# zendesk/min-tfs-client

Hardware: NVIDIA H100
Metric: TensorProto encode+decode GB/s (higher is better)
Workload: dtype u8

## Files before the change

include/b200tfs.h:

```cpp
#ifndef B200TFS_H_
#define B200TFS_H_

#include <stddef.h>
#include <stdint.h>

#ifdef __cplusplus
extern "C" {
#endif

#define B200TFS_ABI_VERSION 2

#define B200TFS_OK 0
#define B200TFS_E_DTYPE (-1)
#define B200TFS_E_SHAPE (-2)
#define B200TFS_E_SIZE (-3)
#define B200TFS_E_PARSE (-4)
#define B200TFS_E_CUDA (-5)
#define B200TFS_E_TOOBIG (-6)
#define B200TFS_E_ARG (-7)
#define B200TFS_E_NONCANONICAL (-8)
#define B200TFS_E_RANGE (-9)
#define B200TFS_E_KEY (-10)
#define B200TFS_E_SPILL (-11)

// ... 216 lines not shown
  int64_t dims[B200TFS_MAX_RANK];
  uint64_t bytes;
  int32_t status;
  int32_t bad_rec;
  uint8_t pad_bits[16];
} b200tfs_pad_key;
int b200tfs_padded_layout(const void* wire_host, int32_t n, const uint64_t* rec_off, const uint64_t* rec_len, int32_t n_keys,
                          b200tfs_pad_key* keys, int32_t cast);
int b200tfs_decode_padded(b200tfs_ctx* ctx, const void* arena_dev, int32_t n, const uint64_t* rec_off, const uint64_t* rec_len,
                          int32_t n_keys, const b200tfs_pad_key* keys);
int b200tfs_decode_padded_host_async(b200tfs_ctx* ctx, const void* wire_host, int32_t n, const uint64_t* rec_off,
                                     const uint64_t* rec_len, int32_t n_keys, const b200tfs_pad_key* keys);
int b200tfs_padded_results(b200tfs_ctx* ctx, int32_t n, int32_t n_keys, b200tfs_output* outs, b200tfs_model_spec* specs,
                           int32_t* rec_status);

int b200tfs_capture_begin(b200tfs_ctx* ctx);
int b200tfs_capture_end(b200tfs_ctx* ctx, void** graph_exec);
int b200tfs_graph_launch(b200tfs_ctx* ctx, void* graph_exec);
int b200tfs_graph_destroy(void* graph_exec);
int b200tfs_wait_event(b200tfs_ctx* ctx, void* ev);

int b200tfs_encode_requests_host(b200tfs_ctx* ctx, int32_t n, const b200tfs_request* reqs,
                                 void* wire_host, uint64_t wire_cap, uint64_t* rec_off,
                                 uint64_t* rec_len);
int b200tfs_encode_requests_host_async(b200tfs_ctx* ctx, int32_t n, const b200tfs_request* reqs,
                                       void* wire_host, uint64_t wire_cap, uint64_t* rec_off,
                                       uint64_t* rec_len);
int b200tfs_decode_responses_host_async(b200tfs_ctx* ctx, const void* wire_host, int32_t n,
                                        const uint64_t* rec_off, const uint64_t* rec_len,
                                        void* dst_host, uint64_t dst_stride);
int b200tfs_pipelined_calls(b200tfs_ctx* ctx, uint64_t* count);
int b200tfs_direct_calls(b200tfs_ctx* ctx, uint64_t* count);
int b200tfs_set_pipeline(b200tfs_ctx* ctx, uint64_t min_bytes, int32_t max_slices);
int b200tfs_encode_tensor_protos_host(b200tfs_ctx* ctx, int32_t n, const b200tfs_tensor* tensors,
                                      void* wire_host, uint64_t wire_cap, uint64_t* rec_off,
                                      uint64_t* rec_len);
int b200tfs_parse_responses_host(b200tfs_ctx* ctx, const void* wire_host, int32_t n,
                                 const uint64_t* rec_off, const uint64_t* rec_len, int32_t max_outputs,
                                 b200tfs_output* outs, int32_t* n_outs, b200tfs_model_spec* specs,
                                 int32_t* rec_status);
int b200tfs_parse_tensor_protos_host(b200tfs_ctx* ctx, const void* wire_host, int32_t n,
                                     const uint64_t* rec_off, const uint64_t* rec_len,
                                     b200tfs_output* outs, int32_t* rec_status);
int b200tfs_unpack_outputs_host(b200tfs_ctx* ctx, int32_t m, const b200tfs_output* outs,
                                const uint64_t* out_rec_off, void* const* dst_host,
                                const int32_t* dst_dtype, int32_t* status);

#define B200TFS_F_BROADCAST 0x10u
typedef struct b200tfs_feature {
  const void* data;
  int32_t src_dtype;
  uint32_t flags;
  int64_t row_elems;
  const char* key;
  int64_t key_len;
} b200tfs_feature;

typedef struct b200tfs_example_request {
  const char* model_name;
  int64_t model_name_len;
  int32_t has_version;
  int32_t order;
  int64_t version;
  int64_t n_examples;
  int32_t n_features;
  int32_t flags;
// ... 30 lines not shown
```

min-tfs-client_b200/csrc/codec_host.cpp:

```cpp
#include <cuda_runtime.h>
#include <stdarg.h>
#include <stdio.h>
#include <stdlib.h>
#include <string.h>

#include <algorithm>
#include <string>
#include <unordered_map>
#include <vector>

#include "../../include/b200tfs.h"
#include "example_walk.h"
#include "frame.h"
#include "kernels.h"
#include "plan.h"
#include "tpl.h"
#include "walker.h"
#include "wire.h"

using namespace b200tfs;

static thread_local char g_err[512] = "";

static int fail(int code, const char* fmt, ...) {
// ... 32 lines not shown
  int32_t dtype = 0;
  void* tile_val = nullptr;
  void* group_sum = nullptr;
  void* total = nullptr;
};

struct b200tfs_ctx {
  int device = 0;
  int sm_count = 132;
  cudaStream_t stream = nullptr;
  cudaStream_t own_stream = nullptr;
  cudaStream_t aux_stream = nullptr;
  cudaStream_t d2h_stream = nullptr;
  static constexpr int kPipeMax = 8;
  cudaEvent_t pipe_ev[2 * kPipeMax + 2] = {};
  uint64_t pipe_min = 1ull << 20;
  int pipe_max = 4;
  uint64_t pipelined_calls = 0;
  uint64_t direct_calls = 0;
  bool opt_direct_out = true;
  Growable guard_dev;
  uint32_t decode_cast = 0;
  uint32_t decode_varints = 0;
  bool fused_varints = false;
  Growable vdec_dev;
  Slot slots[kSlots];
  int next_slot = 0;
  Growable scratch_dev;
  Growable scratch_host;
  Growable stage_dev;
  Growable arena_dev;
  uint64_t launches = 0;
  uint32_t tile_bytes_override = 0;
  bool capturing = false;
  std::vector<Slot*> graph_slots;
  Growable fused_host;
  void* tpl_dev = nullptr;
  uint32_t tpl_flip = 0;
  TplInline* tpl_pinned = nullptr;
  TplInline tpl_known{};
  uint32_t serial = 0;
  cudaEvent_t tpl_event = nullptr;
  bool tpl_event_pending = false;
  bool opt_no_inline = false;
  uint64_t stage_shift = 0;
  int32_t fused_n = 0;
  std::vector<int32_t> pending_status;
  Growable measured_dev;
  uint64_t measured_used = 0;
  std::unordered_map<const void*, MeasuredTensor> measured;
  Growable spill_dev;
  std::vector<SpillEntry> spill_host;
  uint32_t spill_per_rec = 16;
  uint32_t spill_last_per = 0;
  int32_t spill_last_n = 0;
  Growable gather_dev;
  Growable enc_host;
  int32_t enc_n = 0;
  bool has_graphs = false;
  struct KeyResults {
    int32_t n = 0, k = 0;
    uint8_t* dst[B200TFS_CONCAT_MAX_KEYS] = {};
    uint64_t vouts = 0, vstat = 0, specs = 0, status = 0;
  };
  Growable concat_dev;
  KeyResults concat_res;
// ... 397 lines not shown

struct VarJob {
  const uint8_t* src;
  uint8_t* dst;
  uint64_t n_elems;
  uint64_t packed_len;
  int32_t src_dtype;
};

struct PlanBuilder {
  std::vector<MoveItem> items;
  std::vector<SmallItem> smalls;
  std::vector<uint8_t> blob;
  std::vector<VarJob> varjobs;
  uint64_t large_bytes = 0;
  const uint32_t* guard = nullptr;
  uint32_t guard_div = 1;
  bool independent = false;

  void header(uint8_t* dst, size_t blob_off, size_t n) {
    while (n) {
      uint32_t k = (uint32_t)std::min<size_t>(n, kSmallMax);
      smalls.push_back(SmallItem{(uint64_t)blob_off, dst, k, OP_COPY | OP_FLAG_BLOB, 0, 0});
      dst += k; blob_off += k; n -= k;
    }
  }
  void payload(const uint8_t* src, uint8_t* dst, uint64_t n_out, uint32_t op, uint32_t glen = 0, uint32_t gstride = 0) {
    if (!n_out) return;
    if (n_out <= kSmallMax) smalls.push_back(SmallItem{(uint64_t)(uintptr_t)src, dst, (uint32_t)n_out, op, glen, gstride});
    else { items.push_back(MoveItem{src, dst, n_out, op, 0, glen, gstride}); large_bytes += n_out; }
  }
};

uint32_t pick_vec_per_tile(const b200tfs_ctx* c, uint64_t large_bytes, uint64_t max_tile = 65536) {
  uint64_t tile = c->tile_bytes_override;
  if (!tile) {
    uint64_t target_tiles = (uint64_t)c->sm_count * 8;
    tile = (large_bytes + target_tiles - 1) / target_tiles;
    tile = (tile + 32767) & ~32767ull;
    tile = std::min<uint64_t>(std::max<uint64_t>(tile, 32768), max_tile);
  }
  tile = std::max<uint64_t>(tile & ~31ull, 32);
  return (uint32_t)(tile / 16);
}

struct BuiltPlan {
  PlanHeader ph{};
  uint8_t inline_buf[kInlinePlanBytes];
  const uint8_t* host_img = nullptr;
  uint8_t* plan_dev = nullptr;
  uint64_t image = 0;
  Slot* slot = nullptr;
};

int build_plan(b200tfs_ctx* c, PlanBuilder& pb, bool force_dev, BuiltPlan* bp) {
  const uint32_t vpt = pick_vec_per_tile(c, pb.large_bytes);
  uint64_t n_tiles = 0;
  uint32_t uniform = 0;
  bool is_uniform = !pb.items.empty();
  for (auto& it : pb.items) {
    uint64_t t = tiles_for_host(it.n_out, vpt);
    if (n_tiles + t > 0x7FFFFFFFull) return fail(B200TFS_E_TOOBIG, "batch needs more than 2^31 tiles");
    it.n_tiles = (uint32_t)t;
    if (&it == &pb.items[0]) uniform = (uint32_t)t; else if (t != uniform) is_uniform = false;
    n_tiles += t;
  }
  if (!is_uniform) uniform = 0;
  PlanHeader& ph = bp->ph;
  ph = PlanHeader{};
  ph.n_items = (uint32_t)pb.items.size();
  ph.n_tiles = (uint32_t)n_tiles;
  ph.n_small = (uint32_t)pb.smalls.size();
  ph.uniform_tpi = uniform;
  ph.vec_per_tile = vpt;
  ph.guard = pb.guard; ph.guard_div = pb.guard_div ? pb.guard_div : 1u;
  ph.independent = pb.independent ? 1u : 0u;
  const PlanGeometry g = plan_geometry(pb.items.size(), uniform ? 0 : n_tiles, pb.smalls.size());
  ph.off_items = (uint32_t)g.off_items; ph.off_tiles = (uint32_t)g.off_tiles; ph.off_small = (uint32_t)g.off_small;
  Layout P{g.end};
  const uint64_t off_blob = P.take(pb.blob.size(), 1);
  const uint64_t image = P.take(0);
  if (image > 0xFFFFFFFFull) return fail(B200TFS_E_TOOBIG, "plan image larger than 4 GiB");
  bp->image = image;
  uint8_t* img;
  const bool inl = !force_dev && image <= kInlinePlanBytes;
  if (inl) img = bp->inline_buf;
  else {
    int rc = claim_slot(c, image, &bp->slot);
    if (rc) return rc;
    img = (uint8_t*)bp->slot->host.p;
  }
  bp->host_img = img;
  memcpy(img, &ph, sizeof ph);
  if (!pb.items.empty()) memcpy(img + ph.off_items, pb.items.data(), pb.items.size() * sizeof(MoveItem));
  if (!uniform && n_tiles) {
    TileRef* tr = (TileRef*)(img + ph.off_tiles);
    uint32_t g = 0;
    for (uint32_t i = 0; i < pb.items.size(); ++i)
      for (uint32_t t = 0; t < pb.items[i].n_tiles; ++t) tr[g++] = TileRef{i, t};
  }
  SmallItem* sm = (SmallItem*)(img + ph.off_small);
  for (size_t i = 0; i < pb.smalls.size(); ++i) {
    sm[i] = pb.smalls[i];
    if (sm[i].op & OP_FLAG_BLOB) sm[i].src += off_blob;
  }
  if (!pb.blob.empty()) memcpy(img + off_blob, pb.blob.data(), pb.blob.size());
  if (!inl) {
    int rc = upload_slot(c, bp->slot, image);
    if (rc) return rc;
    bp->plan_dev = (uint8_t*)bp->slot->dev.p;
  }
  return B200TFS_OK;
}

int launch_built_plan(b200tfs_ctx* c, BuiltPlan& bp) {
  CU(launch_move(bp.plan_dev, bp.host_img, (uint32_t)bp.image, bp.ph.n_tiles, bp.ph.n_small, c->stream));
  c->launches += 1;
  if (bp.slot && bp.slot->done && !c->capturing) { CU(cudaEventRecord(bp.slot->done, c->stream)); bp.slot->pending = true; }
  return B200TFS_OK;
}

int launch_plan(b200tfs_ctx* c, PlanBuilder& pb) {
  if (pb.items.empty() && pb.smalls.empty()) return B200TFS_OK;
  BuiltPlan bp;
  int rc = build_plan(c, pb, false, &bp);
  if (rc) return rc;
  return launch_built_plan(c, bp);
}

inline uint64_t place_record(uint64_t cursor, uint64_t largest_payload_off) {
  uint64_t slot = (cursor + 255) & ~255ull;
  uint64_t pad = (128 - (largest_payload_off & 127)) & 127;
  return slot + pad;
}

int plan_tensor(const b200tfs_tensor& t, const TensorLayout& L, uint8_t* dst_payload, PlanBuilder& pb) {
  if (!L.payload_len) return B200TFS_OK;
  if (L.varint) {
    pb.varjobs.push_back(VarJob{(const uint8_t*)t.data, dst_payload, L.n_elems, L.payload_len, t.src_dtype});
    return B200TFS_OK;
  }
  pb.payload((const uint8_t*)t.data, dst_payload, L.payload_len, L.op);
  return B200TFS_OK;
}

int run_varjobs(b200tfs_ctx* c, PlanBuilder& pb);

struct RequestLayout {
  std::vector<TensorLayout> tl;
// ... 1189 lines not shown
    if (direct) c->direct_calls += 1;
    else for (int i = 0; i < n; ++i) rec_off[i] -= lo;
    return B200TFS_OK;
  }
  if ((rc = grow_dev(c, c->arena_dev, need))) return rc;
  if ((rc = b200tfs_encode_requests(c, n, rq.data(), c->arena_dev.p, c->arena_dev.cap, rec_off, rec_len))) return rc;
  const uint64_t lo = rec_off[0], hi = rec_off[n - 1] + rec_len[n - 1];
  if (hi - lo > wire_cap) return fail(B200TFS_E_SIZE, "wire buffer too small: need %llu bytes", (unsigned long long)(hi - lo));
  CU(cudaMemcpyAsync(wire_host, (uint8_t*)c->arena_dev.p + lo, hi - lo, cudaMemcpyDeviceToHost, c->stream));
  for (int i = 0; i < n; ++i) rec_off[i] -= lo;
  return B200TFS_OK;
}

int b200tfs_pipelined_calls(b200tfs_ctx* c, uint64_t* count) {
  if (!c || !count) return fail(B200TFS_E_ARG, "bad arguments");
  *count = c->pipelined_calls;
  return B200TFS_OK;
}

int b200tfs_direct_calls(b200tfs_ctx* c, uint64_t* count) {
  if (!c || !count) return fail(B200TFS_E_ARG, "bad arguments");
  *count = c->direct_calls;
  return B200TFS_OK;
}

int b200tfs_set_pipeline(b200tfs_ctx* c, uint64_t min_bytes, int32_t max_slices) {
  if (!c) return fail(B200TFS_E_ARG, "ctx is NULL");
  if (min_bytes && (max_slices < 2 || max_slices > b200tfs_ctx::kPipeMax)) return fail(B200TFS_E_ARG, "max_slices must be in [2, %d]", b200tfs_ctx::kPipeMax);
  c->pipe_min = min_bytes;
  if (min_bytes) c->pipe_max = max_slices;
  return B200TFS_OK;
}

int b200tfs_encode_requests_host(b200tfs_ctx* c, int32_t n, const b200tfs_request* reqs, void* wire_host, uint64_t wire_cap,
                                 uint64_t* rec_off, uint64_t* rec_len) {
  int rc = b200tfs_encode_requests_host_async(c, n, reqs, wire_host, wire_cap, rec_off, rec_len);
  if (rc) return rc;
  CU(cudaStreamSynchronize(c->stream));
  return B200TFS_OK;
}

static int stage_wire(b200tfs_ctx* c, const void* wire_host, int32_t n, const uint64_t* rec_off, const uint64_t* rec_len, uint64_t* span,
                      uint64_t shift = 0, bool copy = true) {
  uint64_t hi = 0;
  for (int i = 0; i < n; ++i) hi = std::max(hi, rec_off[i] + rec_len[i]);
  int rc = grow_dev(c, c->stage_dev, hi + 64);
  if (rc) return rc;
  c->stage_shift = shift;
  if (hi && copy) CU(cudaMemcpyAsync((uint8_t*)c->stage_dev.p + shift, wire_host, hi, cudaMemcpyHostToDevice, c->stream));
  *span = hi;
  return B200TFS_OK;
}

int b200tfs_parse_responses_host(b200tfs_ctx* c, const void* wire_host, int32_t n, const uint64_t* rec_off, const uint64_t* rec_len,
                                 int32_t max_outputs, b200tfs_output* outs, int32_t* n_outs, b200tfs_model_spec* specs,
                                 int32_t* rec_status) {
  if (!c || n < 0 || (n && (!wire_host || !rec_off || !rec_len))) return fail(B200TFS_E_ARG, "bad arguments");
  if (n == 0) return B200TFS_OK;
  CU(cudaSetDevice(c->device));
  uint64_t span;
  int rc = stage_wire(c, wire_host, n, rec_off, rec_len, &span);
  if (rc) return rc;
  return parse_common(c, c->stage_dev.p, n, rec_off, rec_len, max_outputs, false, outs, n_outs, specs, rec_status);
}

int b200tfs_parse_tensor_protos_host(b200tfs_ctx* c, const void* wire_host, int32_t n, const uint64_t* rec_off, const uint64_t* rec_len,
// ... 220 lines not shown
ConcatLayout concat_layout(uint64_t n, uint64_t n_keys, uint64_t tile_cap, uint64_t var_tile_cap) {
  const PlanGeometry g = plan_geometry(n * n_keys * B200TFS_MAX_RUNS, tile_cap, 0);
  const VarPlanLayout V = var_plan_layout(n, var_tile_cap);
  Layout R;
  ConcatLayout L;
  L.outs = R.take(sizeof(b200tfs_output) * n * (kFusedMaxOutputs + 1), 256);
  L.nouts = R.take(4 * n, 256);
  L.specs = R.take(sizeof(b200tfs_model_spec) * n, 256);
  L.status = R.take(4 * n, 256);
  L.spill = R.take(4 * n, 256);
  L.kst = R.take(4 * n * n_keys, 256);
  L.match = R.take(4 * n * n_keys, 256);
  L.plan = R.take(g.end, 256);
  L.plan_tiles = g.off_tiles;
  L.vouts = R.take(sizeof(b200tfs_output) * n * kFusedMaxOutputs, 256);
  L.vnouts = R.take(4 * n, 256);
  L.vstatus = R.take(4 * n, 256);
  L.var = R.take(V.bytes, 256);
  L.var_status = L.var + V.status;
  L.bytes = R.end;
  return L;
}
}

int b200tfs_decode_concat(b200tfs_ctx* c, const void* arena_dev, int32_t n, const uint64_t* rec_off, const uint64_t* rec_len,
                          int32_t n_keys, const b200tfs_concat_key* keys) {
  if (!c || n <= 0 || !arena_dev || !rec_off || !rec_len) return fail(B200TFS_E_ARG, "bad arguments");
  int rc = concat_check_keys(n_keys, keys);
  if (rc) return rc;
  for (int k = 0; k < n_keys; ++k) if (keys[k].dst_cap && !keys[k].dst) return fail(B200TFS_E_ARG, "key %d: dst is NULL", k);
  if (!c->capturing) CU(cudaSetDevice(c->device));
  uint64_t wire_total = 0, tile_cap = 0, var_tile_cap = 0;
  for (int i = 0; i < n; ++i) wire_total += rec_len[i];
  const uint32_t vpt = pick_vec_per_tile(c, c->decode_cast ? wire_total / 2 : wire_total);
  for (int i = 0; i < n; ++i) {
    tile_cap += concat_record_tile_bound(rec_len[i], 16ull * vpt, (uint32_t)n_keys);
    var_tile_cap += var_record_tile_bound(rec_len[i]);
  }
  if (tile_cap > 0x7FFFFFFFull || var_tile_cap > 0x7FFFFFFFull) return fail(B200TFS_E_TOOBIG, "batch needs more than 2^31 tiles");
  const ConcatLayout L = concat_layout((uint64_t)n, (uint64_t)n_keys, tile_cap, var_tile_cap);
  if (L.plan_tiles > 0xFFFFFFFFull) return fail(B200TFS_E_TOOBIG, "plan image larger than 4 GiB");
  if ((rc = grow_dev(c, c->concat_dev, L.bytes))) return rc;
  uint64_t key_bytes = 0;
  for (int k = 0; k < n_keys; ++k) key_bytes += (uint64_t)keys[k].key_len;
  Layout K;
  const uint64_t o_off = K.take(8ull * n), o_len = K.take(8ull * n), o_keys = K.take(sizeof(ConcatKeyDev) * n_keys), o_kb = K.take(key_bytes);
  Slot* slot;
  uint8_t* sd;
  rc = upload_image(c, K.end, {{o_off, rec_off, 8ull * n}, {o_len, rec_len, 8ull * n}}, &sd, &slot, [&](uint8_t* h, uint8_t* dev) {
    uint64_t at = o_kb;
    for (int k = 0; k < n_keys; ++k) {
      ConcatKeyDev kd{dev + at, (uint8_t*)keys[k].dst, keys[k].dst_cap, (uint32_t)keys[k].key_len, 0u};
      memcpy(h + o_keys + sizeof(ConcatKeyDev) * k, &kd, sizeof kd);
      if (keys[k].key_len) memcpy(h + at, keys[k].key, (size_t)keys[k].key_len);
      at += (uint64_t)keys[k].key_len;
    }
  });
  if (rc) return rc;
  for (int k = 0; k < n_keys; ++k) c->concat_res.dst[k] = (uint8_t*)keys[k].dst;
  uint8_t* d = (uint8_t*)c->concat_dev.p;
  const uint64_t* off_dev = (const uint64_t*)(sd + o_off);
  CU(launch_parse_responses((const uint8_t*)arena_dev, off_dev, (const uint64_t*)(sd + o_len), n, kFusedMaxOutputs, (b200tfs_output*)(d + L.outs),
                            (int32_t*)(d + L.nouts), (b200tfs_model_spec*)(d + L.specs), (int32_t*)(d + L.status), nullptr, 0u,
                            (uint32_t*)(d + L.spill), c->stream));
  ConcatPlan cp{};
  cp.w = (const uint8_t*)arena_dev; cp.rec_off = off_dev; cp.outs = (const b200tfs_output*)(d + L.outs);
  cp.n_outs = (const int32_t*)(d + L.nouts); cp.rec_status = (const int32_t*)(d + L.status);
// ... 185 lines not shown
```

min-tfs-client_b200/csrc/kernels.cu:

```cuda
#include <cuda_bf16.h>
#include <cuda_fp16.h>
#include <cuda_runtime.h>
#include <stdint.h>
#include <stdlib.h>
#include <string.h>

#include <algorithm>
#include <utility>

#include "frame.h"
#include "kernels.h"
#include "plan.h"
#include "tpl.h"
#include "example_walk.h"
#include "walker.h"
#include "wire.h"

namespace b200tfs {

__device__ __forceinline__ uint4 ld_stream(const uint8_t* p) {
  uint4 r;
  asm volatile("ld.global.nc.L1::no_allocate.v4.u32 {%0,%1,%2,%3}, [%4];"
               : "=r"(r.x), "=r"(r.y), "=r"(r.z), "=r"(r.w) : "l"(p));
  return r;
}
__device__ __forceinline__ uint4 ld_reuse(const uint8_t* p) {
  uint4 r;
  asm volatile("ld.global.nc.v4.u32 {%0,%1,%2,%3}, [%4];"
               : "=r"(r.x), "=r"(r.y), "=r"(r.z), "=r"(r.w) : "l"(p));
  return r;
}
__device__ __forceinline__ void st_stream(uint8_t* p, const uint4& v) {
  asm volatile("st.global.L1::no_allocate.v4.u32 [%0], {%1,%2,%3,%4};"
               :: "l"(p), "r"(v.x), "r"(v.y), "r"(v.z), "r"(v.w) : "memory");
}

__device__ __forceinline__ void pdl_launch_dependents() { asm volatile("griddepcontrol.launch_dependents;" ::: "memory"); }
__device__ __forceinline__ void pdl_wait_prior_grids() { asm volatile("griddepcontrol.wait;" ::: "memory"); }

__device__ __forceinline__ uint32_t bool_norm_word(uint32_t w) {
  uint32_t t = ((w & 0x7F7F7F7Fu) + 0x7F7F7F7Fu) | w;
  return (t >> 7) & 0x01010101u;
}

template <uint32_t OP>
__device__ __forceinline__ uint4 fix_vec(uint4 v) {
  if (OP == OP_QUIET_SRC || OP == OP_QUIET_DST) {
    v.x = quiet_f32(v.x); v.y = quiet_f32(v.y); v.z = quiet_f32(v.z); v.w = quiet_f32(v.w);
  } else if (OP == OP_BOOL) {
    v.x = bool_norm_word(v.x); v.y = bool_norm_word(v.y); v.z = bool_norm_word(v.z); v.w = bool_norm_word(v.w);
  }
  return v;
}

template <int Q>
__device__ __forceinline__ uint4 shift_pair(const uint4& lo, const uint4& hi, uint32_t s) {
  const uint32_t w[8] = {lo.x, lo.y, lo.z, lo.w, hi.x, hi.y, hi.z, hi.w};
  uint4 o;
  o.x = __funnelshift_r(w[Q + 0], w[Q + 1], s);
  o.y = __funnelshift_r(w[Q + 1], w[Q + 2], s);
  o.z = __funnelshift_r(w[Q + 2], w[Q + 3], s);
  o.w = __funnelshift_r(w[Q + 3], w[Q + 4], s);
  return o;
}

__device__ __forceinline__ uint32_t ld_u32_bytes(const uint8_t* p) {
  return (uint32_t)p[0] | ((uint32_t)p[1] << 8) | ((uint32_t)p[2] << 16) | ((uint32_t)p[3] << 24);
// ... 154 lines not shown
    case 1: return body_shifted_q<OP, 1>(S, dst, n, s, mid);
    case 2: return body_shifted_q<OP, 2>(S, dst, n, s, mid);
    default: return body_shifted_q<OP, 3>(S, dst, n, s, mid);
  }
}

template <bool BF>
__device__ __forceinline__ void body_widen(const uint8_t* __restrict__ src, uint8_t* __restrict__ dst, uint32_t units) {
  constexpr uint32_t kU = 8;
  for (uint32_t base = 0; base < units; base += kU * kMoveThreads) {
    uint4 h[kU];
#pragma unroll
    for (uint32_t i = 0; i < kU; ++i) {
      const uint32_t u = base + i * kMoveThreads + threadIdx.x;
      h[i] = make_uint4(0, 0, 0, 0);
      if (u < units) h[i] = ld_stream(src + 16ull * u);
    }
#pragma unroll
    for (uint32_t i = 0; i < kU; ++i) {
      const uint32_t u = base + i * kMoveThreads + threadIdx.x;
      if (u < units) {
        const uint4 x = h[i];
        uint4 lo, hi;
        if (BF) {
          lo.x = widen_bf16(x.x & 0xFFFF); lo.y = widen_bf16(x.x >> 16); lo.z = widen_bf16(x.y & 0xFFFF); lo.w = widen_bf16(x.y >> 16);
          hi.x = widen_bf16(x.z & 0xFFFF); hi.y = widen_bf16(x.z >> 16); hi.z = widen_bf16(x.w & 0xFFFF); hi.w = widen_bf16(x.w >> 16);
        } else {
          lo.x = widen_f16(x.x & 0xFFFF); lo.y = widen_f16(x.x >> 16); lo.z = widen_f16(x.y & 0xFFFF); lo.w = widen_f16(x.y >> 16);
          hi.x = widen_f16(x.z & 0xFFFF); hi.y = widen_f16(x.z >> 16); hi.z = widen_f16(x.w & 0xFFFF); hi.w = widen_f16(x.w >> 16);
        }
        st_stream(dst + 32ull * u, lo);
        st_stream(dst + 32ull * u + 16, hi);
      }
    }
  }
}

template <bool BF>
__device__ __forceinline__ uint32_t narrow2(uint32_t a, uint32_t b) {
  return BF ? (f32_bits_to_bf16_bits(a) | (f32_bits_to_bf16_bits(b) << 16))
            : (f32_bits_to_f16_bits(a) | (f32_bits_to_f16_bits(b) << 16));
}
template <bool BF, int Q, class Mid>
__device__ __forceinline__ bool body_narrow_q(const uint8_t* __restrict__ S, uint8_t* __restrict__ dst, uint32_t n, uint32_t s, bool aligned, Mid& mid) {
  constexpr uint32_t kU = 4, kRun = 32 * kU, kRound = kRun * (kMoveThreads / 32);
  const uint32_t lane = threadIdx.x & 31, warp = threadIdx.x >> 5;
  for (uint32_t base = 0; base < n; base += kRound) {
    const uint32_t run = base + warp * kRun;
    const uint32_t run_end = min(run + kRun, n);
    uint4 a[kU], b[kU], extra = make_uint4(0, 0, 0, 0);
#pragma unroll
    for (uint32_t i = 0; i < kU; ++i) {
      const uint32_t u = run + 32 * i + lane;
      a[i] = b[i] = make_uint4(0, 0, 0, 0);
      if (u < n) { const uint8_t* p = S + 32ull * u; a[i] = ld_stream(p); b[i] = ld_stream(p + 16); }
    }
    if (!aligned && lane == 0 && run < n) extra = ld_stream(S + 32ull * run_end);
    if (base == 0 && !mid()) return false;
    extra = shfl_lane0(extra);
#pragma unroll
    for (uint32_t i = 0; i < kU; ++i) {
      const uint32_t u = run + 32 * i + lane;
      uint4 c = shfl_down1(a[i]);
      if (i + 1 < kU) {
        const uint4 nxt = shfl_lane0(a[i + 1]);
        if (lane == 31) c = nxt;
// ... 95 lines not shown
        case OP_QUIET_SRC: go = body_same_width<OP_QUIET_SRC>(src_body + 16 * v0, d, n, mid); break;
        case OP_QUIET_DST: go = body_same_width<OP_QUIET_DST>(src_body + 16 * v0, d, n, mid); break;
        case OP_H2F: go = mid(); if (go) body_widen<false>(src_body + 8 * v0, d, n >> 1); break;
        case OP_B2F: go = mid(); if (go) body_widen<true>(src_body + 8 * v0, d, n >> 1); break;
        case OP_F2H: go = body_narrow<false>(src_body + 32 * v0, d, n, mid); break;
        default: go = body_narrow<true>(src_body + 32 * v0, d, n, mid); break;
      }
    }
  } else go = mid();
  if (!go) return false;
  if (tile == 0) for (uint64_t i = threadIdx.x; i < head; i += blockDim.x) dst[i] = gen_byte(op, src, i);
  if (last) for (uint64_t i = head + (nvec << 4) + threadIdx.x; i < n_out; i += blockDim.x) dst[i] = gen_byte(op, src, i);
  return true;
}

__device__ __noinline__ void move_tile_cold(const uint8_t* src, uint8_t* dst, uint64_t n_out, uint32_t op, uint32_t n_tiles, uint32_t tile,
                                            uint32_t vpt) {
  AlwaysGo go;
  move_tile<true>(src, dst, n_out, op, n_tiles, tile, vpt, go);
}

__device__ __noinline__ void move_tile_narrow(const uint8_t* src, uint8_t* dst, uint64_t n_out, uint32_t op, uint32_t n_tiles, uint32_t tile,
                                              uint32_t vpt) {
  AlwaysGo go;
  move_tile<false>(src, dst, n_out, op, n_tiles, tile, vpt, go);
}
__device__ __forceinline__ bool op_narrows(uint32_t op) { return op == OP_F2H || op == OP_F2B; }

struct GuardMid {
  uint32_t g;
  __device__ __forceinline__ bool operator()() const { return g != 0; }
};

template <bool GUARD>
__device__ __forceinline__ void move_body(const uint8_t* plan) {
  const PlanHeader& ph = *reinterpret_cast<const PlanHeader*>(plan);
  const uint32_t b = blockIdx.x;
  if (b < ph.n_tiles) {
    uint32_t item, tile;
    if (ph.uniform_tpi) { item = b / ph.uniform_tpi; tile = b - item * ph.uniform_tpi; }
    else {
      const TileRef tr = reinterpret_cast<const TileRef*>(plan + ph.off_tiles)[b];
      item = tr.item; tile = tr.tile;
    }
    const MoveItem& it = reinterpret_cast<const MoveItem*>(plan + ph.off_items)[item];
    if (GUARD) {
      GuardMid mid{ph.guard[item / ph.guard_div]};
      if (it.gstride) { if (mid()) move_tile_gather(SrcView{it.src, it.glen, it.gstride}, it.dst, it.n_out, it.op, it.n_tiles, tile, ph.vec_per_tile); return; }
      move_tile<false>(it.src, it.dst, it.n_out, it.op, it.n_tiles, tile, ph.vec_per_tile, mid);
      return;
    }
    if (it.gstride) { move_tile_gather(SrcView{it.src, it.glen, it.gstride}, it.dst, it.n_out, it.op, it.n_tiles, tile, ph.vec_per_tile); return; }
    AlwaysGo go;
    move_tile<false>(it.src, it.dst, it.n_out, it.op, it.n_tiles, tile, ph.vec_per_tile, go);
  } else {
    const uint32_t warps = blockDim.x >> 5;
    const uint32_t idx = (b - ph.n_tiles) * warps + (threadIdx.x >> 5);
    if (idx >= ph.n_small) return;
    const SmallItem si = reinterpret_cast<const SmallItem*>(plan + ph.off_small)[idx];
    const uint32_t op = si.op & ~OP_FLAG_BLOB;
    const SrcView src{(si.op & OP_FLAG_BLOB) ? plan + si.src : reinterpret_cast<const uint8_t*>(si.src), si.glen, si.gstride};
    const uint32_t lane = threadIdx.x & 31;
    for (uint32_t i = lane; i < si.n_out; i += 32) si.dst[i] = gen_byte(op, src, i);
  }
}

__global__ void __launch_bounds__(kMoveThreads, 3) move_kernel(const uint8_t* __restrict__ plan) {
  pdl_launch_dependents();
  if (!reinterpret_cast<const PlanHeader*>(plan)->independent) pdl_wait_prior_grids();
  move_body<false>(plan);
}

__global__ void __launch_bounds__(kMoveThreads, 3) move_kernel_inline(const __grid_constant__ InlinePlan plan) {
  pdl_launch_dependents();
  pdl_wait_prior_grids();
  move_body<false>(plan.bytes);
}

__global__ void __launch_bounds__(kMoveThreads, 3) move_guarded_kernel(const uint8_t* __restrict__ plan) {
  pdl_launch_dependents();
  pdl_wait_prior_grids();
  move_body<true>(plan);
}

__global__ void __launch_bounds__(32) parse_responses_kernel(const uint8_t* __restrict__ w, const uint64_t* __restrict__ rec_off,
                                                             const uint64_t* __restrict__ rec_len, int n, int max_outputs,
                                                             b200tfs_output* outs, int32_t* n_outs, b200tfs_model_spec* specs,
                                                             int32_t* status, SpillEntry* spill, uint32_t spill_per_rec, uint32_t* spill_used) {
  __shared__ __align__(16) uint8_t lines[32][256];
  int r = blockIdx.x * blockDim.x + threadIdx.x;
  if (r >= n) return;
  const uint64_t off = rec_off[r], len = rec_len[r];
  spill_used[r] = 0;
  if (len > 0x7FFFFFFFull) { status[r] = B200TFS_E_PARSE; n_outs[r] = 0; return; }
  Cursor c;
  cur_open(c, w + off, (uint32_t)len, lines[threadIdx.x]);
  SpillArea sp{spill_per_rec ? spill + (size_t)r * spill_per_rec : nullptr, spill_per_rec, 0u};
  int cnt = 0;
  b200tfs_output* mine = outs + (size_t)r * (max_outputs + 1);
  status[r] = walk_response(c, max_outputs, mine, &cnt, specs + r, sp);
  for (int k = 0; k < cnt; ++k) mine[k].spill_rec = (uint32_t)r;
  n_outs[r] = cnt;
  spill_used[r] = sp.used;
}

__global__ void __launch_bounds__(32) parse_tensors_kernel(const uint8_t* __restrict__ w, const uint64_t* __restrict__ rec_off,
                                                           const uint64_t* __restrict__ rec_len, int n, b200tfs_output* outs,
                                                           int32_t* status, SpillEntry* spill, uint32_t spill_per_rec, uint32_t* spill_used) {
  __shared__ __align__(16) uint8_t lines[32][256];
// ... 551 lines not shown

cudaError_t launch_frame_requests(const FrameTables& ft, cudaStream_t stream) {
  if (!ft.n) return cudaSuccess;
  frame_requests_kernel<<<(ft.n + kFrameWarps - 1) / kFrameWarps, 32 * kFrameWarps, 0, stream>>>(ft);
  return cudaGetLastError();
}

__global__ void __launch_bounds__(256) fill_edge_kernel(uint8_t* __restrict__ dst, uint32_t elem_size, uint64_t have_imm,
                                                        const unsigned long long* __restrict__ have_dev, uint64_t n_elems) {
  const uint64_t have = have_dev ? (uint64_t)*have_dev : have_imm;
  if (have >= n_elems) return;
  uint8_t last[16];
#pragma unroll
  for (uint32_t b = 0; b < 16; ++b) last[b] = (have && b < elem_size) ? dst[(have - 1) * elem_size + b] : (uint8_t)0;
  for (uint64_t i = have + blockIdx.x * (uint64_t)blockDim.x + threadIdx.x; i < n_elems; i += (uint64_t)gridDim.x * blockDim.x)
#pragma unroll
    for (uint32_t b = 0; b < 16; ++b) if (b < elem_size) dst[i * elem_size + b] = last[b];
}

template <class... KArgs, class... Args>
static cudaError_t launch_pdl(void (*kernel)(KArgs...), uint32_t grid, uint32_t block, uint32_t dyn_smem, cudaStream_t stream, Args&&... args) {
  static const bool env_off = [] { const char* e = getenv("B200TFS_PDL"); return !(e && e[0] == '1'); }();
  const bool off = env_off;
  cudaLaunchConfig_t cfg{};
  cfg.gridDim = dim3(grid); cfg.blockDim = dim3(block); cfg.dynamicSmemBytes = dyn_smem; cfg.stream = stream;
  cudaLaunchAttribute attr[1];
  attr[0].id = cudaLaunchAttributeProgrammaticStreamSerialization;
  attr[0].val.programmaticStreamSerializationAllowed = 1;
  cfg.attrs = attr; cfg.numAttrs = off ? 0 : 1;
  return cudaLaunchKernelEx(&cfg, kernel, std::forward<Args>(args)...);
}

cudaError_t launch_move(const uint8_t* plan_dev, const uint8_t* plan_host, uint32_t plan_bytes, uint32_t n_tiles,
                        uint32_t n_small, cudaStream_t stream) {
  const uint32_t warps = kMoveThreads / 32;
  const uint32_t grid = n_tiles + (n_small + warps - 1) / warps;
  if (grid == 0) return cudaSuccess;
  if (plan_dev == nullptr) {
    InlinePlan ip;
    memcpy(ip.bytes, plan_host, plan_bytes);
    return launch_pdl(move_kernel_inline, grid, kMoveThreads, 0, stream, ip);
  }
  if (!(plan_host && reinterpret_cast<const PlanHeader*>(plan_host)->independent)) return launch_pdl(move_kernel, grid, kMoveThreads, 0, stream, plan_dev);
  cudaLaunchConfig_t cfg{};
  cfg.gridDim = dim3(grid); cfg.blockDim = dim3(kMoveThreads); cfg.dynamicSmemBytes = 0; cfg.stream = stream;
  cudaLaunchAttribute attr[1];
  attr[0].id = cudaLaunchAttributeProgrammaticStreamSerialization;
  attr[0].val.programmaticStreamSerializationAllowed = 1;
  cfg.attrs = attr; cfg.numAttrs = 1;
  return cudaLaunchKernelEx(&cfg, move_kernel, plan_dev);
}

cudaError_t launch_parse_responses(const uint8_t* w, const uint64_t* rec_off, const uint64_t* rec_len, int n, int max_outputs,
                                   b200tfs_output* outs, int32_t* n_outs, b200tfs_model_spec* specs, int32_t* status,
                                   void* spill, uint32_t spill_per_rec, uint32_t* spill_used, cudaStream_t stream) {
  if (n <= 0) return cudaSuccess;
  parse_responses_kernel<<<(n + 31) / 32, 32, 0, stream>>>(w, rec_off, rec_len, n, max_outputs, outs, n_outs, specs, status,
                                                          (SpillEntry*)spill, spill_per_rec, spill_used);
  return cudaGetLastError();
}

cudaError_t launch_parse_tensors(const uint8_t* w, const uint64_t* rec_off, const uint64_t* rec_len, int n, b200tfs_output* outs,
                                 int32_t* status, void* spill, uint32_t spill_per_rec, uint32_t* spill_used, cudaStream_t stream) {
  if (n <= 0) return cudaSuccess;
  parse_tensors_kernel<<<(n + 31) / 32, 32, 0, stream>>>(w, rec_off, rec_len, n, outs, status, (SpillEntry*)spill, spill_per_rec, spill_used);
  return cudaGetLastError();
}

uint32_t tiles_for_host(uint64_t n_out, uint32_t vpt) { return tiles_for(n_out, vpt); }

cudaError_t launch_fill_edge(uint8_t* dst, uint32_t elem_size, uint64_t have, const unsigned long long* have_dev, uint64_t n_elems,
                             cudaStream_t stream) {
  if (!n_elems) return cudaSuccess;
  const uint64_t blocks = std::min<uint64_t>((n_elems + 255) / 256, 132 * 8);
  fill_edge_kernel<<<(uint32_t)blocks, 256, 0, stream>>>(dst, elem_size, have, have_dev, n_elems);
  return cudaGetLastError();
}

cudaError_t launch_decode_fused(const FusedParams& fp, uint32_t grid, cudaStream_t stream) {
  if (!grid) return cudaSuccess;
  {
    static bool opted[64] = {};
    int dev = 0;
// ... 76 lines not shown
```

min-tfs-client_b200/csrc/kernels.h:

```cpp
#pragma once
#include <cuda_runtime.h>
#include <stdint.h>

#include "../../include/b200tfs.h"
#include "plan.h"

namespace b200tfs {

cudaError_t launch_move(const uint8_t* plan_dev, const uint8_t* plan_host, uint32_t plan_bytes, uint32_t n_tiles,
                        uint32_t n_small, cudaStream_t stream);

cudaError_t launch_move_guarded(const uint8_t* plan_dev, uint32_t n_tiles, cudaStream_t stream);

constexpr uint32_t kSpillEntryBytes = 32;
cudaError_t launch_parse_responses(const uint8_t* w, const uint64_t* rec_off, const uint64_t* rec_len, int n, int max_outputs,
                                   b200tfs_output* outs, int32_t* n_outs, b200tfs_model_spec* specs, int32_t* status,
                                   void* spill, uint32_t spill_per_rec, uint32_t* spill_used, cudaStream_t stream);
cudaError_t launch_parse_tensors(const uint8_t* w, const uint64_t* rec_off, const uint64_t* rec_len, int n, b200tfs_output* outs,
                                 int32_t* status, void* spill, uint32_t spill_per_rec, uint32_t* spill_used, cudaStream_t stream);

cudaError_t launch_decode_fused(const FusedParams& fp, uint32_t grid, cudaStream_t stream);
constexpr uint32_t kStageVecsHost = 2048;
uint32_t tiles_for_host(uint64_t n_out, uint32_t vpt);
cudaError_t launch_fill_edge(uint8_t* dst, uint32_t elem_size, uint64_t have, const unsigned long long* have_dev, uint64_t n_elems,
                             cudaStream_t stream);
cudaError_t launch_frame_requests(const FrameTables& ft, cudaStream_t stream);
cudaError_t launch_venc_len(const VarTables& tb, cudaStream_t stream);
cudaError_t launch_venc_emit(const VarTables& tb, cudaStream_t stream);
cudaError_t launch_vdec_count(const VarTables& tb, cudaStream_t stream);
cudaError_t launch_vdec_emit(const VarTables& tb, cudaStream_t stream);
cudaError_t launch_vdec_plan(const VarPlan& vp, cudaStream_t stream);
cudaError_t launch_vdec_dev(const VarTables& tb, uint32_t max_ctas, cudaStream_t stream, const VarPadMap* pm = nullptr);
cudaError_t launch_concat_plan(const ConcatPlan& cp, uint32_t move_grid, cudaStream_t stream);
cudaError_t launch_padded(const PaddedPlan& pp, uint32_t emit_grid, cudaStream_t stream);
cudaError_t launch_example_requests(const ExTables& T, cudaStream_t stream, uint32_t* launched);
cudaError_t launch_example_responses(const XrTables& T, uint32_t emit_ctas, cudaStream_t stream, uint32_t* launched);

}
```

min-tfs-client_b200/min_tfs_client/_native.py:

```python
from __future__ import annotations

import ctypes as C
import os
import threading

import numpy as np

_HERE = os.path.dirname(os.path.abspath(__file__))
LIB_PATH = os.environ.get("B200TFS_LIB") or os.path.join(os.path.dirname(_HERE), "lib", "libb200tfs.so")

OK = 0
E_DTYPE, E_SHAPE, E_SIZE, E_PARSE, E_CUDA, E_TOOBIG, E_ARG, E_NONCANONICAL, E_RANGE, E_KEY, E_SPILL = range(-1, -12, -1)

F_TENSOR_CONTENT = 0x1
F_KEEP_SNAN = 0x2
F_PRESERIALIZED = 0x4
F_DEVICE_DATA = 0x8
RF_GRPC_FRAME = 0x1
OF_TENSOR_CONTENT, OF_MULTI_CHUNK, OF_DIM_INFERRED, OF_HAS_UNKNOWN, OF_RANK0, OF_VARINT, OF_PAD_EDGE = 0x1, 0x2, 0x4, 0x8, 0x10, 0x20, 0x40
OF_UNPACKED, OF_SPILLED, OF_DEVICE_VARINT = 0x80, 0x100, 0x200
ORDER_GIVEN, ORDER_UPB, ORDER_BYTES = 0, 1, 2
MAX_RANK, MAX_RUNS, FUSED_MAX_OUTPUTS, CONCAT_MAX_KEYS = 16, 8, 8, 8
DT_HALF_REFQUIRK = -19

# ... 124 lines not shown
    "b200tfs_encode_tensor_protos": (C.c_int, [_vp, C.c_int32, C.POINTER(Tensor), _vp, C.c_uint64, _u64p, _u64p]),
    "b200tfs_encode_requests": (C.c_int, [_vp, C.c_int32, C.POINTER(Request), _vp, C.c_uint64, _u64p, _u64p]),
    "b200tfs_encode_requests_async": (C.c_int, [_vp, C.c_int32, C.POINTER(Request), _vp, C.c_uint64]),
    "b200tfs_encode_results": (C.c_int, [_vp, C.c_int32, _u64p, _u64p]),
    "b200tfs_request_frame_deferred": (C.c_int, [C.POINTER(Request), _u64p, _vp, C.c_uint64, _u64p, _u64p, _u64p, _u64p]),
    "b200tfs_parse_responses": (C.c_int, [_vp, _vp, C.c_int32, _u64p, _u64p, C.c_int32, C.POINTER(Output), _i32p,
                                          C.POINTER(ModelSpec), _i32p]),
    "b200tfs_parse_tensor_protos": (C.c_int, [_vp, _vp, C.c_int32, _u64p, _u64p, C.POINTER(Output), _i32p]),
    "b200tfs_output_dims": (C.c_int, [_vp, C.POINTER(Output), C.POINTER(C.c_int64), C.c_int32]),
    "b200tfs_output_runs": (C.c_int, [_vp, C.POINTER(Output), C.POINTER(Run), C.c_int32]),
    "b200tfs_unpack_outputs": (C.c_int, [_vp, _vp, C.c_int32, C.POINTER(Output), _u64p, _vpp, _i32p, _i32p]),
    "b200tfs_decode_responses": (C.c_int, [_vp, _vp, C.c_int32, _u64p, _u64p, _vp, C.c_uint64]),
    "b200tfs_decode_results": (C.c_int, [_vp, C.c_int32, C.POINTER(Output), _i32p, C.POINTER(ModelSpec), _i32p]),
    "b200tfs_decode_stats": (C.c_int, [_vp, _u64p, _u64p, _u64p]),
    "b200tfs_concat_layout": (C.c_int, [_vp, C.c_int32, _u64p, _u64p, C.c_int32, C.POINTER(ConcatKey), C.c_int32]),
    "b200tfs_response_keys": (C.c_int, [_vp, C.c_uint64, C.c_int32, _u64p, C.POINTER(C.c_uint32), _i32p]),
    "b200tfs_decode_concat": (C.c_int, [_vp, _vp, C.c_int32, _u64p, _u64p, C.c_int32, C.POINTER(ConcatKey)]),
    "b200tfs_decode_concat_host_async": (C.c_int, [_vp, _vp, C.c_int32, _u64p, _u64p, C.c_int32, C.POINTER(ConcatKey)]),
    "b200tfs_concat_results": (C.c_int, [_vp, C.c_int32, C.c_int32, C.POINTER(Output), C.POINTER(ModelSpec), _i32p]),
    "b200tfs_padded_layout": (C.c_int, [_vp, C.c_int32, _u64p, _u64p, C.c_int32, C.POINTER(PadKey), C.c_int32]),
    "b200tfs_decode_padded": (C.c_int, [_vp, _vp, C.c_int32, _u64p, _u64p, C.c_int32, C.POINTER(PadKey)]),
    "b200tfs_decode_padded_host_async": (C.c_int, [_vp, _vp, C.c_int32, _u64p, _u64p, C.c_int32, C.POINTER(PadKey)]),
    "b200tfs_padded_results": (C.c_int, [_vp, C.c_int32, C.c_int32, C.POINTER(Output), C.POINTER(ModelSpec), _i32p]),
    "b200tfs_capture_begin": (C.c_int, [_vp]),
    "b200tfs_capture_end": (C.c_int, [_vp, _vpp]),
    "b200tfs_graph_launch": (C.c_int, [_vp, _vp]),
    "b200tfs_graph_destroy": (C.c_int, [_vp]),
    "b200tfs_wait_event": (C.c_int, [_vp, _vp]),
    "b200tfs_encode_requests_host": (C.c_int, [_vp, C.c_int32, C.POINTER(Request), _vp, C.c_uint64, _u64p, _u64p]),
    "b200tfs_encode_requests_host_async": (C.c_int, [_vp, C.c_int32, C.POINTER(Request), _vp, C.c_uint64, _u64p, _u64p]),
    "b200tfs_pipelined_calls": (C.c_int, [_vp, _u64p]),
    "b200tfs_direct_calls": (C.c_int, [_vp, _u64p]),
    "b200tfs_set_pipeline": (C.c_int, [_vp, C.c_uint64, C.c_int32]),
    "b200tfs_set_decode_cast": (C.c_int, [_vp, C.c_int32]),
    "b200tfs_set_decode_varints": (C.c_int, [_vp, C.c_int32]),
    "b200tfs_decode_slot_bytes": (C.c_int, [_vp, C.c_int32, _u64p, _u64p, C.c_int32, _u64p, _i32p]),
    "b200tfs_decode_responses_host_async": (C.c_int, [_vp, _vp, C.c_int32, _u64p, _u64p, _vp, C.c_uint64]),
    "b200tfs_encode_tensor_protos_host": (C.c_int, [_vp, C.c_int32, C.POINTER(Tensor), _vp, C.c_uint64, _u64p, _u64p]),
    "b200tfs_parse_responses_host": (C.c_int, [_vp, _vp, C.c_int32, _u64p, _u64p, C.c_int32, C.POINTER(Output), _i32p,
                                               C.POINTER(ModelSpec), _i32p]),
    "b200tfs_parse_tensor_protos_host": (C.c_int, [_vp, _vp, C.c_int32, _u64p, _u64p, C.POINTER(Output), _i32p]),
    "b200tfs_unpack_outputs_host": (C.c_int, [_vp, C.c_int32, C.POINTER(Output), _u64p, _vpp, _i32p, _i32p]),
    "b200tfs_example_request_size": (C.c_int, [C.POINTER(ExampleRequest), _u64p]),
    "b200tfs_example_arena_size": (C.c_int, [C.c_int32, C.POINTER(ExampleRequest), _u64p]),
    "b200tfs_encode_example_requests_async": (C.c_int, [_vp, C.c_int32, C.POINTER(ExampleRequest), _vp, C.c_uint64]),
    "b200tfs_encode_example_requests_host": (C.c_int, [_vp, C.c_int32, C.POINTER(ExampleRequest), _vp, C.c_uint64, _u64p, _u64p]),
    "b200tfs_example_response_bound": (C.c_int, [C.c_int32, C.c_int32, _u64p, _u64p, _u64p]),
    "b200tfs_decode_example_responses": (C.c_int, [_vp, C.c_int32, _vp, C.c_int32, _u64p, _u64p, _vp, C.c_uint64, _vp, C.c_uint64]),
    "b200tfs_decode_example_responses_host_async": (C.c_int, [_vp, C.c_int32, _vp, C.c_int32, _u64p, _u64p, _vp, C.c_uint64, _vp,
                                                              C.c_uint64]),
    "b200tfs_example_response_results": (C.c_int, [_vp, C.c_int32, C.POINTER(C.c_int64), C.POINTER(ModelSpec), C.POINTER(C.c_int64)]),
}

_lib = None
_lib_lock = threading.Lock()


def load():
    global _lib
    if _lib is not None:
        return _lib
    with _lib_lock:
        if _lib is not None:
            return _lib
        if not os.path.exists(LIB_PATH):
            raise RuntimeError(
# ... 64 lines not shown
```

Baseline: 1429.

## Add dedicated widen kernel for half/bf16-to-float moves and cap plan tile size

```diff
diff --git a/include/b200tfs.h b/include/b200tfs.h
--- a/include/b200tfs.h
+++ b/include/b200tfs.h
@@ -272,6 +272,7 @@
 int b200tfs_pipelined_calls(b200tfs_ctx* ctx, uint64_t* count);
 int b200tfs_direct_calls(b200tfs_ctx* ctx, uint64_t* count);
 int b200tfs_set_pipeline(b200tfs_ctx* ctx, uint64_t min_bytes, int32_t max_slices);
+int b200tfs_set_widen_route(b200tfs_ctx* ctx, int32_t on);
 int b200tfs_encode_tensor_protos_host(b200tfs_ctx* ctx, int32_t n, const b200tfs_tensor* tensors,
                                       void* wire_host, uint64_t wire_cap, uint64_t* rec_off,
                                       uint64_t* rec_len);
diff --git a/min-tfs-client_b200/csrc/codec_host.cpp b/min-tfs-client_b200/csrc/codec_host.cpp
--- a/min-tfs-client_b200/csrc/codec_host.cpp
+++ b/min-tfs-client_b200/csrc/codec_host.cpp
@@ -88,6 +88,7 @@
   Growable arena_dev;
   uint64_t launches = 0;
   uint32_t tile_bytes_override = 0;
+  bool widen_route = true;
   bool capturing = false;
   std::vector<Slot*> graph_slots;
   Growable fused_host;
@@ -551,7 +552,7 @@
   }
 };
 
-uint32_t pick_vec_per_tile(const b200tfs_ctx* c, uint64_t large_bytes, uint64_t max_tile = 65536) {
+uint32_t pick_vec_per_tile(const b200tfs_ctx* c, uint64_t large_bytes, uint64_t max_tile) {
   uint64_t tile = c->tile_bytes_override;
   if (!tile) {
     uint64_t target_tiles = (uint64_t)c->sm_count * 8;
@@ -570,10 +571,11 @@
   uint8_t* plan_dev = nullptr;
   uint64_t image = 0;
   Slot* slot = nullptr;
+  bool widen = false;
 };
 
 int build_plan(b200tfs_ctx* c, PlanBuilder& pb, bool force_dev, BuiltPlan* bp) {
-  const uint32_t vpt = pick_vec_per_tile(c, pb.large_bytes);
+  const uint32_t vpt = pick_vec_per_tile(c, pb.large_bytes, 32768);
   uint64_t n_tiles = 0;
   uint32_t uniform = 0;
   bool is_uniform = !pb.items.empty();
@@ -583,6 +585,7 @@
     it.n_tiles = (uint32_t)t;
     if (&it == &pb.items[0]) uniform = (uint32_t)t; else if (t != uniform) is_uniform = false;
     n_tiles += t;
+    if ((it.op == OP_H2F || it.op == OP_B2F) && !it.gstride) bp->widen = c->widen_route;
   }
   if (!is_uniform) uniform = 0;
   PlanHeader& ph = bp->ph;
@@ -633,7 +636,7 @@
 }
 
 int launch_built_plan(b200tfs_ctx* c, BuiltPlan& bp) {
-  CU(launch_move(bp.plan_dev, bp.host_img, (uint32_t)bp.image, bp.ph.n_tiles, bp.ph.n_small, c->stream));
+  CU(launch_move(bp.plan_dev, bp.host_img, (uint32_t)bp.image, bp.ph.n_tiles, bp.ph.n_small, bp.widen, c->stream));
   c->launches += 1;
   if (bp.slot && bp.slot->done && !c->capturing) { CU(cudaEventRecord(bp.slot->done, c->stream)); bp.slot->pending = true; }
   return B200TFS_OK;
@@ -1889,6 +1892,13 @@
   return B200TFS_OK;
 }
 
+int b200tfs_set_widen_route(b200tfs_ctx* c, int32_t on) {
+  if (!c) return fail(B200TFS_E_ARG, "ctx is NULL");
+  if (on != 0 && on != 1) return fail(B200TFS_E_ARG, "on must be 0 or 1");
+  c->widen_route = on != 0;
+  return B200TFS_OK;
+}
+
 int b200tfs_encode_requests_host(b200tfs_ctx* c, int32_t n, const b200tfs_request* reqs, void* wire_host, uint64_t wire_cap,
                                  uint64_t* rec_off, uint64_t* rec_len) {
   int rc = b200tfs_encode_requests_host_async(c, n, reqs, wire_host, wire_cap, rec_off, rec_len);
@@ -2175,7 +2185,7 @@
   if (!c->capturing) CU(cudaSetDevice(c->device));
   uint64_t wire_total = 0, tile_cap = 0, var_tile_cap = 0;
   for (int i = 0; i < n; ++i) wire_total += rec_len[i];
-  const uint32_t vpt = pick_vec_per_tile(c, c->decode_cast ? wire_total / 2 : wire_total);
+  const uint32_t vpt = pick_vec_per_tile(c, c->decode_cast ? wire_total / 2 : wire_total, 65536);
   for (int i = 0; i < n; ++i) {
     tile_cap += concat_record_tile_bound(rec_len[i], 16ull * vpt, (uint32_t)n_keys);
     var_tile_cap += var_record_tile_bound(rec_len[i]);
diff --git a/min-tfs-client_b200/csrc/kernels.cu b/min-tfs-client_b200/csrc/kernels.cu
--- a/min-tfs-client_b200/csrc/kernels.cu
+++ b/min-tfs-client_b200/csrc/kernels.cu
@@ -33,6 +33,11 @@
 __device__ __forceinline__ void st_stream(uint8_t* p, const uint4& v) {
   asm volatile("st.global.L1::no_allocate.v4.u32 [%0], {%1,%2,%3,%4};"
                :: "l"(p), "r"(v.x), "r"(v.y), "r"(v.z), "r"(v.w) : "memory");
+}
+__device__ __forceinline__ uint2 ld_stream64(const uint8_t* p) {
+  uint2 r;
+  asm volatile("ld.global.nc.L1::no_allocate.v2.u32 {%0,%1}, [%2];" : "=r"(r.x), "=r"(r.y) : "l"(p));
+  return r;
 }
 
 __device__ __forceinline__ void pdl_launch_dependents() { asm volatile("griddepcontrol.launch_dependents;" ::: "memory"); }
@@ -253,6 +258,32 @@
         st_stream(dst + 32ull * u, lo);
         st_stream(dst + 32ull * u + 16, hi);
       }
+    }
+  }
+}
+
+template <bool BF>
+__device__ __forceinline__ uint4 widen_vec(const uint2& x) {
+  uint4 o;
+  if (BF) { o.x = widen_bf16(x.x & 0xFFFF); o.y = widen_bf16(x.x >> 16); o.z = widen_bf16(x.y & 0xFFFF); o.w = widen_bf16(x.y >> 16); }
+  else { o.x = widen_f16(x.x & 0xFFFF); o.y = widen_f16(x.x >> 16); o.z = widen_f16(x.y & 0xFFFF); o.w = widen_f16(x.y >> 16); }
+  return o;
+}
+template <bool BF>
+__device__ __forceinline__ void body_widen_lines(const uint8_t* __restrict__ src, uint8_t* __restrict__ dst, uint32_t n) {
+  constexpr uint32_t kV = 16;
+  for (uint32_t base = 0; base < n; base += kV * kMoveThreads) {
+    uint2 h[kV];
+#pragma unroll
+    for (uint32_t i = 0; i < kV; ++i) {
+      const uint32_t v = base + i * kMoveThreads + threadIdx.x;
+      h[i] = make_uint2(0, 0);
+      if (v < n) h[i] = ld_stream64(src + 8ull * v);
+    }
+#pragma unroll
+    for (uint32_t i = 0; i < kV; ++i) {
+      const uint32_t v = base + i * kMoveThreads + threadIdx.x;
+      if (v < n) st_stream(dst + 16ull * v, widen_vec<BF>(h[i]));
     }
   }
 }
@@ -414,7 +445,20 @@
   __device__ __forceinline__ bool operator()() const { return g != 0; }
 };
 
-template <bool GUARD>
+__device__ __forceinline__ bool move_tile_widen(const uint8_t* __restrict__ src, uint8_t* __restrict__ dst, uint64_t n_out, uint32_t op,
+                                                uint32_t n_tiles, uint32_t tile, uint32_t vpt) {
+  if ((op != OP_H2F && op != OP_B2F) || (((uintptr_t)src | (uintptr_t)dst) & 15)) return false;
+  const uint64_t nvec = (n_out >> 5) << 1, v0 = (uint64_t)tile * vpt;
+  if (v0 < nvec) {
+    const uint32_t n = (uint32_t)min((uint64_t)vpt, nvec - v0);
+    if (op == OP_H2F) body_widen_lines<false>(src + 8 * v0, dst + 16 * v0, n);
+    else body_widen_lines<true>(src + 8 * v0, dst + 16 * v0, n);
+  }
+  if (tile + 1 == n_tiles) for (uint64_t i = (nvec << 4) + threadIdx.x; i < n_out; i += blockDim.x) dst[i] = gen_byte(op, src, i);
+  return true;
+}
+
+template <bool GUARD, bool WIDEN = false>
 __device__ __forceinline__ void move_body(const uint8_t* plan) {
   const PlanHeader& ph = *reinterpret_cast<const PlanHeader*>(plan);
   const uint32_t b = blockIdx.x;
@@ -433,6 +477,11 @@
       return;
     }
     if (it.gstride) { move_tile_gather(SrcView{it.src, it.glen, it.gstride}, it.dst, it.n_out, it.op, it.n_tiles, tile, ph.vec_per_tile); return; }
+    if (WIDEN) {
+      if (!move_tile_widen(it.src, it.dst, it.n_out, it.op, it.n_tiles, tile, ph.vec_per_tile))
+        move_tile_narrow(it.src, it.dst, it.n_out, it.op, it.n_tiles, tile, ph.vec_per_tile);
+      return;
+    }
     AlwaysGo go;
     move_tile<false>(it.src, it.dst, it.n_out, it.op, it.n_tiles, tile, ph.vec_per_tile, go);
   } else {
@@ -457,6 +506,18 @@
   pdl_launch_dependents();
   pdl_wait_prior_grids();
   move_body<false>(plan.bytes);
+}
+
+__global__ void __launch_bounds__(kMoveThreads, 2) move_widen_kernel(const uint8_t* __restrict__ plan) {
+  pdl_launch_dependents();
+  if (!reinterpret_cast<const PlanHeader*>(plan)->independent) pdl_wait_prior_grids();
+  move_body<false, true>(plan);
+}
+
+__global__ void __launch_bounds__(kMoveThreads, 2) move_widen_kernel_inline(const __grid_constant__ InlinePlan plan) {
+  pdl_launch_dependents();
+  pdl_wait_prior_grids();
+  move_body<false, true>(plan.bytes);
 }
 
 __global__ void __launch_bounds__(kMoveThreads, 3) move_guarded_kernel(const uint8_t* __restrict__ plan) {
@@ -1074,23 +1135,24 @@
 }
 
 cudaError_t launch_move(const uint8_t* plan_dev, const uint8_t* plan_host, uint32_t plan_bytes, uint32_t n_tiles,
-                        uint32_t n_small, cudaStream_t stream) {
+                        uint32_t n_small, bool widen, cudaStream_t stream) {
   const uint32_t warps = kMoveThreads / 32;
   const uint32_t grid = n_tiles + (n_small + warps - 1) / warps;
   if (grid == 0) return cudaSuccess;
   if (plan_dev == nullptr) {
     InlinePlan ip;
     memcpy(ip.bytes, plan_host, plan_bytes);
-    return launch_pdl(move_kernel_inline, grid, kMoveThreads, 0, stream, ip);
-  }
-  if (!(plan_host && reinterpret_cast<const PlanHeader*>(plan_host)->independent)) return launch_pdl(move_kernel, grid, kMoveThreads, 0, stream, plan_dev);
+    return launch_pdl(widen ? move_widen_kernel_inline : move_kernel_inline, grid, kMoveThreads, 0, stream, ip);
+  }
+  void (*const kernel)(const uint8_t*) = widen ? move_widen_kernel : move_kernel;
+  if (!(plan_host && reinterpret_cast<const PlanHeader*>(plan_host)->independent)) return launch_pdl(kernel, grid, kMoveThreads, 0, stream, plan_dev);
   cudaLaunchConfig_t cfg{};
   cfg.gridDim = dim3(grid); cfg.blockDim = dim3(kMoveThreads); cfg.dynamicSmemBytes = 0; cfg.stream = stream;
   cudaLaunchAttribute attr[1];
   attr[0].id = cudaLaunchAttributeProgrammaticStreamSerialization;
   attr[0].val.programmaticStreamSerializationAllowed = 1;
   cfg.attrs = attr; cfg.numAttrs = 1;
-  return cudaLaunchKernelEx(&cfg, move_kernel, plan_dev);
+  return cudaLaunchKernelEx(&cfg, kernel, plan_dev);
 }
 
 cudaError_t launch_parse_responses(const uint8_t* w, const uint64_t* rec_off, const uint64_t* rec_len, int n, int max_outputs,
diff --git a/min-tfs-client_b200/csrc/kernels.h b/min-tfs-client_b200/csrc/kernels.h
--- a/min-tfs-client_b200/csrc/kernels.h
+++ b/min-tfs-client_b200/csrc/kernels.h
@@ -8,7 +8,7 @@
 namespace b200tfs {
 
 cudaError_t launch_move(const uint8_t* plan_dev, const uint8_t* plan_host, uint32_t plan_bytes, uint32_t n_tiles,
-                        uint32_t n_small, cudaStream_t stream);
+                        uint32_t n_small, bool widen, cudaStream_t stream);
 
 cudaError_t launch_move_guarded(const uint8_t* plan_dev, uint32_t n_tiles, cudaStream_t stream);
 
diff --git a/min-tfs-client_b200/min_tfs_client/_native.py b/min-tfs-client_b200/min_tfs_client/_native.py
--- a/min-tfs-client_b200/min_tfs_client/_native.py
+++ b/min-tfs-client_b200/min_tfs_client/_native.py
@@ -180,6 +180,7 @@
     "b200tfs_pipelined_calls": (C.c_int, [_vp, _u64p]),
     "b200tfs_direct_calls": (C.c_int, [_vp, _u64p]),
     "b200tfs_set_pipeline": (C.c_int, [_vp, C.c_uint64, C.c_int32]),
+    "b200tfs_set_widen_route": (C.c_int, [_vp, C.c_int32]),
     "b200tfs_set_decode_cast": (C.c_int, [_vp, C.c_int32]),
     "b200tfs_set_decode_varints": (C.c_int, [_vp, C.c_int32]),
     "b200tfs_decode_slot_bytes": (C.c_int, [_vp, C.c_int32, _u64p, _u64p, C.c_int32, _u64p, _i32p]),
```

Result: faster. 1449, median of 6 (+1.4%).
